# ska-sa/katsdpsigproc

Measured on AMD Instinct MI355X. Metric: visibility samples/s (baselines x channels) through full RFI flagger, higher is better.
Workload: dtype f32 amplitude / f64 deviations

## Files before the change

katsdpsigproc_amd/csrc/fused_common.h:

```cpp
#pragma once
#include <stdlib.h>

#include "bitplane.h"
#include "median_merge.h"
#include "median_window.h"

#ifndef FUSED_MAD_BITS
#define FUSED_MAD_BITS 1
#endif
#ifndef FUSED_STRIP
#define FUSED_STRIP 4
#endif
#define FUSED_THREADS (64 * FUSED_STRIP)
#define FUSED_MAD_NORMAL 1.4826

#ifdef KSP_DIAG_REALTIME
#define FUSED_DIAG_CLOCK() __builtin_amdgcn_s_memrealtime()
#else
#define FUSED_DIAG_CLOCK() __builtin_amdgcn_s_memtime()
#endif
#ifdef KSP_DIAG
#define FUSED_DIAG_STOP(p) ((p).debug_stop)
#define FUSED_DIAG_TRACE(p) ((p).trace)
#else
// ... 516 lines not shown
                                            int tiny = 0)
{
    static_assert(!HAVE_EXACT || R == 64, "exactness masks are 64 bits, one per sample of a lane");
    constexpr int NP = R / 2;
    const int c0 = lane * R;
    auto dv = [&](int j) -> float {
        float x = dev[j];
        asm("" : "+v"(x));
        return x;
    };
    unsigned kp[NP];
#pragma unroll
    for (int i = 0; i < NP; i++) {
        const unsigned a = __float_as_uint(dev[2 * i]) + 0xffffu;
        const unsigned b = __float_as_uint(dev[2 * i + 1]) + 0xffffu;
        kp[i] = __builtin_amdgcn_perm(b, a, 0x07060302u) & 0x7fff7fffu;
    }
    int zeros;
    if constexpr (R != 64) zeros = count_less16<NP>(kp, 1);
    auto stamp = [&](int i) {
        if (trace != nullptr && lane == 0) trace[i] = FUSED_DIAG_CLOCK();
    };
    stamp(8);
    if (debug_stop == 31) return (double)(kp[0] + kp[NP - 1]);
    const int total = 64 * R;
    unsigned K = 0;
    int below_bin = 0, in_bin;
    int rank2 = 0, rank = 0;
    int zeros_keys = 0;
    unsigned eq0 = 0, eq1 = 0;
    if constexpr (R == 64) {
        unsigned np[32];
#pragma unroll
        for (int i = 0; i < 32; i++) np[i] = kp[i] ^ 0x7fff7fffu;
        transpose_bits32(np);
        stamp(9);
        {
            unsigned z0 = np[0], z1 = np[16];
#pragma unroll
            for (int b = 1; b < 15; b++) {
                z0 &= np[b];
                z1 &= np[16 + b];
            }
            zeros = ksp_wave_sum_dpp(__popc(z0) + __popc(z1));
        }
        zeros_keys = zeros;
        if (ksp_any(tiny != 0)) zeros -= ksp_wave_sum_dpp(tiny);
        if (zeros == total) return __builtin_nan("");
        rank2 = total + zeros;
        rank = rank2 / 2;
        if (rank < zeros_keys) return 0x1p-150 * FUSED_MAD_NORMAL;
        eq0 = eq1 = 0xffffffffu;
        auto step2 = [&](int hi, int lo) {
            const unsigned a0 = eq0 & np[hi], a1 = eq1 & np[16 + hi];
            const unsigned z00_0 = a0 & np[lo], z00_1 = a1 & np[16 + lo];
            const unsigned z01_0 = a0 ^ z00_0, z01_1 = a1 ^ z00_1;
            const unsigned b0 = eq0 ^ a0, b1 = eq1 ^ a1;
            const unsigned z10_0 = b0 & np[lo], z10_1 = b1 & np[16 + lo];
            const unsigned z11_0 = b0 ^ z10_0, z11_1 = b1 ^ z10_1;
            int s01 = (__popc(z00_0) + __popc(z00_1)) | ((__popc(z01_0) + __popc(z01_1)) << 16);
            int c10 = __popc(z10_0) + __popc(z10_1);
            ksp_wave_sum2_dpp(s01, c10);
            const int n1 = below_bin + (s01 & 0xffff), n2 = n1 + (s01 >> 16), n3 = n2 + c10;
            const bool g1 = n1 <= rank, g2 = n2 <= rank, g3 = n3 <= rank;
            K |= (unsigned)((int)g1 + (int)g2 + (int)g3) << lo;
            below_bin = g3 ? n3 : g2 ? n2 : g1 ? n1 : below_bin;
            eq0 = g3 ? z11_0 : g2 ? z10_0 : g1 ? z01_0 : z00_0;
            eq1 = g3 ? z11_1 : g2 ? z10_1 : g1 ? z01_1 : z00_1;
        };
        auto step1 = [&](int bit) {
            const unsigned z0 = eq0 & np[bit], z1 = eq1 & np[16 + bit];
            const int c = below_bin + ksp_wave_sum_dpp(__popc(z0) + __popc(z1));
            const bool take = c <= rank;
            K |= take ? (1u << bit) : 0u;
            below_bin = take ? c : below_bin;
            eq0 = take ? (eq0 ^ z0) : z0;
            eq1 = take ? (eq1 ^ z1) : z1;
        };
#if FUSED_MAD_BITS == 1
        bool hinted = false;
        if (top_hint != nullptr && *top_hint >= 0) {
            const unsigned h = (unsigned)*top_hint;
            unsigned e0 = 0xffffffffu, e1 = 0xffffffffu;
            int lb = 0;
#pragma unroll
            for (int bit = 14; bit >= 7; bit--) {
                const unsigned z0 = e0 & np[bit], z1 = e1 & np[16 + bit];
                if ((h >> (bit - 7)) & 1) {
                    lb += __popc(z0) + __popc(z1);
                    e0 ^= z0;
                    e1 ^= z1;
                } else {
                    e0 = z0;
                    e1 = z1;
                }
            }
            int cnt = __popc(e0) + __popc(e1);
            ksp_wave_sum2_dpp(lb, cnt);
            if (lb <= rank && rank < lb + cnt) {
                hinted = true;
                K = h << 7;
                below_bin = lb;
                eq0 = e0;
                eq1 = e1;
            }
        }
        if (hinted) {
#pragma unroll
            for (int bit = 6; bit >= 0; bit--) step1(bit);
        } else {
#pragma unroll
            for (int bit = 14; bit >= 0; bit--) step1(bit);
        }
        if (top_hint != nullptr) *top_hint = (int)(K >> 7);
#else
#pragma unroll
        for (int bit = 14; bit >= 2; bit -= 2) step2(bit, bit - 1);
        step1(0);
#endif
        in_bin = ksp_wave_sum_dpp(__popc(eq0) + __popc(eq1));
    } else {
        zeros_keys = zeros;
        if (ksp_any(tiny != 0)) zeros -= ksp_wave_sum(tiny);
        if (zeros == total) return __builtin_nan("");
        rank2 = total + zeros;
        rank = rank2 / 2;
        if (rank < zeros_keys) return 0x1p-150 * FUSED_MAD_NORMAL;
        for (int bit = 14; bit >= 0; bit--) {
            const unsigned test = K | (1u << bit);
            const int c = count_less16<NP>(kp, test);
            if (c <= rank) {
                K = test;
                below_bin = c;
            }
        }
        in_bin = count_less16<NP>(kp, K + 1) - below_bin;
    }
    const bool even = !(rank2 & 1);
    stamp(10);
    if (debug_stop == 32) return (double)(K + below_bin);
    auto key_of = [&](int j) -> unsigned {
        return min((__float_as_uint(dv(j)) & 0x7fffffffu) + 0xffffu, 0x7fffffffu) >> 16;
    };
    auto bin_mask = [&](unsigned key) -> unsigned long long {
        unsigned long long m = 0;
#pragma unroll
        for (int j = 0; j < R; j++)
            if (key_of(j) == key) m |= 1ull << j;
        return m;
    };
    int r = rank - below_bin;
    unsigned long long cand = 0;
    const bool narrowed = in_bin > LIST_CAP;
    if (narrowed) {
        const unsigned first = ((K - 1) << 16) + 1u;
        unsigned offs = 0;
        int below = below_bin;
        for (int bit = 15; bit >= 0; bit--) {
            const unsigned test = first + (offs | (1u << bit));
            int c = 0;
#pragma unroll
            for (int j = 0; j < R; j++) c += (__float_as_uint(dv(j)) & 0x7fffffffu) < test;
            c = ksp_wave_sum(c);
            if (c <= rank) {
                offs |= 1u << bit;
                below = c;
            }
        }
        const unsigned cur = first + offs;
        cand = 0;
#pragma unroll
        for (int j = 0; j < R; j++)
            if ((__float_as_uint(dv(j)) & 0x7fffffffu) == cur) cand |= 1ull << j;
        in_bin = ksp_wave_sum(__popcll(cand));
        r = rank - below;
        below_bin = below;
        if (in_bin > LIST_CAP) {
            auto each = [&](auto &&f) {
                unsigned long long todo = cand;
                while (__any(todo != 0)) {
                    const bool has = todo != 0;
                    const int j = has ? __ffsll((long long)todo) - 1 : 0;
                    todo &= todo - 1;
                    const double x = fabs(exact_dev<WIDTH>(c0 + j, fetch));
                    if (has) f(x);
                }
            };
            double lo = __builtin_inf(), hi = 0.0;
            each([&](double x) {
                lo = fmin(lo, x);
                hi = fmax(hi, x);
            });
            lo = ksp_wave_min(lo);
            hi = ksp_wave_max(hi);
            double xk = lo, prev = lo;
            if (lo != hi) {
                const unsigned long long base = (unsigned long long)__double_as_longlong(lo);
                const unsigned long long span = (unsigned long long)__double_as_longlong(hi) - base;
                unsigned long long offs = 0;
                int below_k = 0;
                for (int bit = 63 - __clzll((long long)span); bit >= 0; bit--) {
                    const unsigned long long test = base + (offs | (1ull << bit));
                    int c = 0;
                    each([&](double x) {
                        c += (unsigned long long)__double_as_longlong(x) < test;
                    });
                    c = ksp_wave_sum(c);
                    if (c <= r) {
                        offs |= 1ull << bit;
                        below_k = c;
                    }
                }
                xk = __longlong_as_double((long long)(base + offs));
                prev = xk;
                if (even && r >= 1 && below_k == r) {
                    double m = 0.0;
                    each([&](double x) { m = (x < xk) ? fmax(m, x) : m; });
                    prev = ksp_wave_max(m);
                }
            }
            if (even && r == 0) {
                float b32 = 0.0f;
#pragma unroll
                for (int j = 0; j < R; j++) {
                    const float a = fabsf(dv(j));
                    b32 = (__float_as_uint(a) < cur) ? fmaxf(b32, a) : b32;
                }
                b32 = ksp_wave_max(b32);
                unsigned long long bm = 0;
#pragma unroll
                for (int j = 0; j < R; j++)
                    if (fabsf(dv(j)) == b32) bm |= 1ull << j;
                const int n2 = gather_exact<WIDTH>(bm, c0, list, 0, LIST_CAP, fetch);
                double below_max = 0.0;
                for (int i = lane; i < min(n2, LIST_CAP); i += 64) below_max = fmax(below_max, list[i]);
                below_max = ksp_wave_max(below_max);
                __builtin_amdgcn_wave_barrier();
                if (n2 > LIST_CAP) {
                    unsigned long long todo = bm;
                    double m = 0.0;
                    while (__any(todo != 0)) {
                        const bool has = todo != 0;
                        const int j = has ? __ffsll((long long)todo) - 1 : 0;
                        todo &= todo - 1;
                        const double x = fabs(exact_dev<WIDTH>(c0 + j, fetch));
                        m = has ? fmax(m, x) : m;
                    }
                    below_max = ksp_wave_max(m);
                }
                prev = below_max;
            }
            if (even) xk = (xk + prev) / 2.0;
            return xk * FUSED_MAD_NORMAL;
        }
    }
    double xk, prev;
    bool have_prev;
    if (!narrowed && in_bin <= 64) {
        int *lc = (int *)list;
        int n = 0;
        auto place = [&](bool hit, int channel) {
            const unsigned long long m = ksp_ballot(hit);
            const int pos = n + __builtin_amdgcn_mbcnt_hi((unsigned)(m >> 32),
                                                         __builtin_amdgcn_mbcnt_lo((unsigned)m, 0));
            if (hit) lc[pos] = channel;
            n += __popcll(m);
        };
        double x;
        bool ranked = false;
        unsigned *lv = (unsigned *)lc + 128;
        static_assert(LIST_CAP * 2 >= 128 + 64 + 8, "candidate values behind the channel numbers");
        if constexpr (R == 64 && HAVE_EXACT) {
            const int mine = __popc(eq0) + __popc(eq1);
            const int incl = ksp_wave_scan_dpp(mine);
            n = __builtin_amdgcn_readlane(incl, 63);
            int pos = incl - mine;
            unsigned h0 = eq0, h1 = eq1;
            while (ksp_any((h0 | h1) != 0)) {
                const bool has = (h0 | h1) != 0;
                int j = 0;
                if (h0) {
                    j = 2 * (__ffs((int)h0) - 1);
                    h0 &= h0 - 1;
                } else if (h1) {
                    j = 2 * (__ffs((int)h1) - 1) + 1;
                    h1 &= h1 - 1;
                }
                const float v = ksp_select_dev<R>(dev, j);
                if (has) {
                    lc[pos] = (c0 + j) | (((exact >> j) & 1) ? (int)0x80000000 : 0);
                    lv[pos] = __float_as_uint(v) & 0x7fffffffu;
                    pos++;
                }
            }
            if (lane < 8) lv[n + lane] = 0xffffffffu;
            __builtin_amdgcn_fence(__ATOMIC_RELEASE, "wavefront");
            __builtin_amdgcn_wave_barrier();
            const int slot = lane < n ? lane : 0;
            const int e0 = lc[slot];
            const unsigned a32 = lv[slot];
            x = (double)__uint_as_float(a32);
            const bool inexact = lane < n && e0 >= 0;
            stamp(11);
            if (debug_stop == 33) return x;
            if (ksp_any(inexact)) {
                const double xe = fabs(exact_dev<WIDTH>(e0 & 0x7fffffff, fetch));
                x = inexact ? xe : x;
            } else {
                unsigned k32, p32;
                rank_list_u32(lv, a32, n, r, lane, k32, p32, have_prev);
                xk = (double)__uint_as_float(k32);
                prev = (double)__uint_as_float(p32);
                ranked = true;
            }
        } else {
            if constexpr (R == 64) {
                const int mine = __popc(eq0) + __popc(eq1);
                const int incl = ksp_wave_scan_dpp(mine);
                n = __builtin_amdgcn_readlane(incl, 63);
                int pos = incl - mine;
                unsigned h0 = eq0, h1 = eq1;
                while (h0 | h1) {
                    if (h0) {
                        lc[pos++] = c0 + 2 * (__ffs((int)h0) - 1);
                        h0 &= h0 - 1;
                    } else {
                        lc[pos++] = c0 + 2 * (__ffs((int)h1) - 1) + 1;
                        h1 &= h1 - 1;
                    }
                }
            } else {
#pragma unroll
                for (int j = 0; j < R; j++) place(key_of(j) == K, c0 + j);
            }
            __builtin_amdgcn_fence(__ATOMIC_RELEASE, "wavefront");
            __builtin_amdgcn_wave_barrier();
            const int c = lc[lane < n ? lane : 0];
            stamp(11);
            if (debug_stop == 33) return (double)c;
            x = fabs(exact_dev<WIDTH>(c, fetch));
        }
        stamp(12);
        if (!ranked) rank_lanes64(x, n, r, lane, xk, prev, have_prev);
        stamp(13);
        __builtin_amdgcn_wave_barrier();
    } else {
        gather_exact<WIDTH>(narrowed ? cand : bin_mask(K), c0, list, 0, LIST_CAP, fetch);
        rank_in_list(list, in_bin, r, lane, xk, prev, have_prev);
        __builtin_amdgcn_wave_barrier();
    }
    if (even && !have_prev) {
        int k2 = -1;
#pragma unroll
        for (int j = 0; j < R; j++) {
            const int kj = (int)key_of(j);
            k2 = (kj < (int)K) ? max(k2, kj) : k2;
        }
        k2 = wave_max_int(k2);
        const bool below_is_tiny = k2 <= 0;
        unsigned long long bm = bin_mask((unsigned)(below_is_tiny ? 0 : k2));
        float b32 = 0.0f;
#pragma unroll
        for (int j = 0; j < R; j++)
            if ((bm >> j) & 1) b32 = fmaxf(b32, fabsf(dv(j)));
        b32 = ksp_wave_max(b32);
        unsigned long long top = 0;
#pragma unroll
        for (int j = 0; j < R; j++)
            if (((bm >> j) & 1) && fabsf(dv(j)) == b32) top |= 1ull << j;
        bool recompute = true;
        if (below_is_tiny) {
            prev = 0x1p-150;
            recompute = false;
        }
        if constexpr (HAVE_EXACT) {
            if (recompute && !ksp_any((top & ~exact) != 0)) {
                prev = (double)b32;
                recompute = false;
            }
        }
        if (recompute) {
            const int n2 = gather_exact<WIDTH>(top, c0, list, 0, LIST_CAP, fetch);
            double below_max = 0.0;
            for (int i = lane; i < min(n2, LIST_CAP); i += 64) below_max = fmax(below_max, list[i]);
            prev = ksp_wave_max(below_max);
            __builtin_amdgcn_wave_barrier();
            if (n2 > LIST_CAP) {
                double m = 0.0;
                while (__any(top != 0)) {
                    const bool has = top != 0;
                    const int j = has ? __ffsll((long long)top) - 1 : 0;
                    top &= top - 1;
                    const double x = fabs(exact_dev<WIDTH>(c0 + j, fetch));
                    m = has ? fmax(m, x) : m;
                }
                prev = ksp_wave_max(m);
            }
        }
    }
    stamp(14);
    if (even) xk = (xk + prev) / 2.0;
    return xk * FUSED_MAD_NORMAL;
}

template <int WIDTH, class Fetch>
__device__ __noinline__ double exact_dev_call(int c, Fetch fetch)
{
    return exact_dev<WIDTH>(c, fetch);
}

template <int WIDTH, class Fetch>
__device__ __forceinline__ unsigned long long threshold_wide(const FusedParams &p,
                                                             const float (&dev)[64],
                                                             unsigned long long fl,
                                                             unsigned long long ge, double t1,
                                                             bool positive, int lane, int C,
                                                             Fetch &&fetch)
{
    const int c0 = lane * 64;
    float nmax = 0.0f;
#pragma unroll
    for (int j = 0; j < 64; j++) nmax = fmaxf(nmax, -dev[j]);
    nmax = ksp_wave_max(nmax);
    float U[64];
    unsigned Nb[16];
#pragma unroll
    for (int j = 0; j < 64; j++) U[j] = dev[j];
#pragma unroll
    for (int q = 0; q < 16; q++) Nb[q] = 0;
    int lvl = -1;
    float umax = 0.0f;
    bool counted = false;
    auto level = [&](auto s_) {
        constexpr int s = decltype(s_)::value;
        ksp_static_for<s>([&](auto r_) {
            constexpr int r = decltype(r_)::value;
            const float e = __shfl_down(U[r], 1, 64);
#pragma unroll
            for (int j = r; j + s < 64; j += s) U[j] += U[j + s];
            U[r + 64 - s] += e;
        });
        if (counted) {
            if constexpr (s >= 4) {
                constexpr int sq = s / 4;
                ksp_static_for<sq>([&](auto r_) {
                    constexpr int r = decltype(r_)::value;
                    const unsigned e = (unsigned)__shfl_down((int)Nb[r], 1, 64);
#pragma unroll
                    for (int q = r; q + sq < 16; q += sq) Nb[q] += Nb[q + sq];
                    Nb[r + 16 - sq] += e;
                });
            } else {
                const unsigned e = (unsigned)__shfl_down((int)Nb[0], 1, 64);
#pragma unroll
                for (int q = 0; q < 16; q++)
                    Nb[q] += __builtin_amdgcn_alignbyte(q + 1 < 16 ? Nb[(q + 1) % 16] : e, Nb[q], s);
            }
        }
    };
#pragma unroll 1
    for (int k = 0; k < p.n_windows; k++) {
        if (positive && !ksp_any((ge & ~fl) != 0)) break;
        const int w = 1 << k;
        const double scale = k == 0 ? p.scales[0] : k == 1 ? p.scales[1] : k == 2 ? p.scales[2]
                           : k == 3 ? p.scales[3] : k == 4 ? p.scales[4] : k == 5 ? p.scales[5]
                           : k == 6 ? p.scales[6] : p.scales[7];
        const float thrf = (float)(t1 * scale);
        const float limf = __fmul_rn(thrf, (float)w);
        const double limit = (double)limf;
        if (positive && lvl >= 0 && umax < thrf) continue;
        if (lvl < 0) {
            counted = ksp_any(fl != 0);
            {
                const unsigned f_lo = (unsigned)fl, f_hi = (unsigned)(fl >> 32);
#pragma unroll
                for (int j = 0; j < 64; j++)
                    U[j] = (((j < 32 ? f_lo : f_hi) >> (j & 31)) & 1u) ? 0.0f : dev[j];
            }
            float m = U[0];
#pragma unroll
            for (int j = 1; j < 64; j++) m = fmaxf(m, U[j]);
            umax = ksp_wave_max(m);
            if (counted) {
#pragma unroll
                for (int q = 0; q < 16; q++)
                    Nb[q] = ((((unsigned)(fl >> (4 * q))) & 0xfu) * 0x00204081u) & 0x01010101u;
            }
            lvl = 0;
            if (positive && umax < thrf) continue;
        }
        while (lvl < k) {
            switch (lvl) {
            case 0: level(std::integral_constant<int, 1>{}); break;
            case 1: level(std::integral_constant<int, 2>{}); break;
            case 2: level(std::integral_constant<int, 4>{}); break;
            case 3: level(std::integral_constant<int, 8>{}); break;
            case 4: level(std::integral_constant<int, 16>{}); break;
            case 5: level(std::integral_constant<int, 32>{}); break;
            default: level(std::integral_constant<int, 64>{}); break;
            }
            lvl++;
        }
        const int nvalid = C - w + 1 - c0;
        const unsigned long long valid = nvalid >= 64 ? ~0ull : nvalid <= 0 ? 0ull : ((1ull << nvalid) - 1);
        unsigned long long hits = 0, unsure = valid;
        if (positive) {
            unsigned h_lo = 0, h_hi = 0, m_lo = 0, m_hi = 0;
            const float c = (float)w * nmax * 0x1p-18f + (float)w * 0x1p-149f;
            if (counted) {
                const unsigned wq = (unsigned)w * 0x01010101u;
                auto one = [&](auto j_, unsigned &h, unsigned &m) {
                    constexpr int j = decltype(j_)::value;
                    const unsigned left = wq - Nb[j / 4];
                    const float rem = (float)((left >> (8 * (j % 4))) & 0xffu);
                    const float T = rem * thrf;
                    const float hi = __builtin_fmaf(T, 1.0f + 0x1p-18f, c);
                    float lo = __builtin_fmaf(T, 1.0f - 0x1p-18f, -c);
                    lo = (rem == 0.0f) ? __builtin_inff() : lo;
                    h = 2 * h + (U[j] > hi);
                    m = 2 * m + (U[j] > lo);
                };
                ksp_static_for<32>([&](auto i_) { one(std::integral_constant<int, 31 - decltype(i_)::value>{}, h_lo, m_lo); });
                ksp_static_for<32>([&](auto i_) { one(std::integral_constant<int, 63 - decltype(i_)::value>{}, h_hi, m_hi); });
            } else {
                const float hi = __builtin_fmaf(limf, 1.0f + 0x1p-18f, c);
                const float lo = __builtin_fmaf(limf, 1.0f - 0x1p-18f, -c);
#pragma unroll
                for (int j = 31; j >= 0; j--) {
                    h_lo = 2 * h_lo + (U[j] > hi);
                    m_lo = 2 * m_lo + (U[j] > lo);
                }
#pragma unroll
                for (int j = 63; j >= 32; j--) {
                    h_hi = 2 * h_hi + (U[j] > hi);
                    m_hi = 2 * m_hi + (U[j] > lo);
                }
            }
            hits = (((unsigned long long)h_hi << 32) | h_lo) & valid;
            unsure = (((unsigned long long)m_hi << 32) | m_lo) & valid & ~hits;
        }
        if (ksp_any(unsure != 0)) {
            const unsigned long long f1 = __shfl_down(fl, 1, 64), f2 = __shfl_down(fl, 2, 64);
            while (ksp_any(unsure != 0)) {
                const bool has = unsure != 0;
                const int j = has ? __ffsll((long long)unsure) - 1 : 0;
                unsure &= unsure - 1;
                double s = 0.0;
                for (int m = 0; m < w; m++) {
                    const int jj = j + m;
                    const unsigned long long fw = jj < 64 ? fl : jj < 128 ? f1 : f2;
                    const bool sub = (fw >> (jj & 63)) & 1;
                    const double x = exact_dev_call<WIDTH>(c0 + jj, fetch);
                    s += sub ? (double)thrf : x;
                }
                if (has && s > limit) hits |= 1ull << j;
            }
            lvl = -1;
        }
        if (!ksp_any(hits != 0)) continue;
        auto suffix_or = [](unsigned long long t) {
            t |= t >> 1; t |= t >> 2; t |= t >> 4; t |= t >> 8; t |= t >> 16; t |= t >> 32;
            return t;
        };
        unsigned long long add = hits;
        for (int s = 1; s < w && s < 64; s <<= 1) add |= add << s;
        unsigned long long h1 = __shfl_up(hits, 1, 64), h2 = __shfl_up(hits, 2, 64);
        if (lane < 1) h1 = 0;
        if (lane < 2) h2 = 0;
        if (w > 64) {
            add |= h1 ? ~0ull : 0ull;
            add |= suffix_or(h2 >> 1);
        } else if (w > 1) {
            add |= suffix_or(h1 >> (65 - w));
        }
        if (ksp_any((add & ~fl) != 0)) {
            fl |= add;
            lvl = -1;
        }
    }
    return fl;
}


template <int R, int WIDTH, int MAXK = 4, class Fetch>
__device__ __forceinline__ unsigned long long threshold_flags(const FusedParams &p,
                                                              const float (&dev)[R], float dmax,
                                                              double noise64, int lane, int C,
                                                              Fetch &&fetch)
{
    static_assert(R <= 64, "flag mask is 64 bits");
    const int c0 = lane * R;
    unsigned long long fl = 0;
    if (p.threshold_kind == KSP_THRESHOLD_SIMPLE) {
        const double thr = p.n_sigma * noise64;
        if (__any((double)dmax * (1.0 + 0x1p-23) > thr)) {
            unsigned long long unsure = 0;
#pragma unroll
            for (int j = 0; j < R; j++) {
                const double d = (double)dev[j];
                const double slack = fabs(d) * 0x1p-23 + 0x1p-149;
                if (d - slack > thr)
                    fl |= 1ull << j;
                else if (d + slack > thr)
                    unsure |= 1ull << j;
            }
            while (__any(unsure != 0)) {
// ... 165 lines not shown
```

katsdpsigproc_amd/csrc/ring_kernel.h:

```cpp
#pragma once
#include "fused_common.h"

#ifndef RING_STOP
#define RING_STOP 0
#endif
#define RING_THREADS 512
#define RING_STRIP 8
#define RING_NSLOT 32
#ifndef RING_G
#define RING_G 4
#endif
#ifndef RING_PRIO
#define RING_PRIO 0
#endif
#ifndef RING_STAGGER
#define RING_STAGGER 0
#endif
#define RING_SLOT_BYTES 4096
#define RING_LIST_DOUBLES 256
#define RING_XCD_GROUP 8

struct RingLayout {
    static constexpr size_t RING_BYTES = (size_t)RING_NSLOT * RING_SLOT_BYTES;
    static constexpr size_t LIST_BYTES = sizeof(double) * RING_LIST_DOUBLES * RING_STRIP;
    static constexpr size_t CTRL_BYTES = 64;
    static constexpr size_t LDS_BYTES = RING_BYTES + LIST_BYTES + CTRL_BYTES;
};

#ifdef RING_TRACE
#define RING_TRACE_STRIPS 24
#define RING_TRACE_SLOTS 16
__device__ unsigned long long ring_trace_buf[256 * 8 * RING_TRACE_STRIPS * RING_TRACE_SLOTS];
#endif

#define RING_WORK_LIST 2
#define RING_WORK_DONE 10

__device__ __forceinline__ int ring_strip_of(int x, int t)
{
    return ((t / RING_XCD_GROUP) * 8 + x) * RING_XCD_GROUP + (t % RING_XCD_GROUP);
}

__device__ __forceinline__ int ring_take(unsigned *work, int x, int n_strips, int t0)
{
    for (int k = 0; k < 8; k++) {
        const int xx = (x + k) & 7;
        const int t = t0 + (int)atomicAdd(&work[RING_WORK_LIST + xx], 1u);
        const int s = ring_strip_of(xx, t);
        if (s < n_strips) return s;
    }
    return -1;
}

__device__ __forceinline__ float ring_from_next(float v, float edge, int lane)
{
    const float r = __shfl_down(v, 1, 64);
    return lane == 63 ? edge : r;
}
__device__ __forceinline__ float ring_from_prev(float v, float edge, int lane)
{
    const float r = __shfl_up(v, 1, 64);
    return lane == 0 ? edge : r;
}

template <int WIDTH>
__global__ __launch_bounds__(RING_THREADS) void flagger_ring_kernel(const FusedParams p)
{
    constexpr int R = 64, W = WIDTH, H = WIDTH / 2;
    constexpr int G = RING_G, NSLOT = RING_NSLOT, STEPS = 64, NCHUNK = STEPS / G;
    constexpr int K = NSLOT / G;
    constexpr int PER_CHUNK = G / 2;
    static_assert(W % 2 == 1 && W <= 13 && 2 * H <= G * 3, "merging median only");
    typedef __attribute__((address_space(3))) void lds_void;
    extern __shared__ __attribute__((aligned(16))) char lds[];
    const int tid = threadIdx.x, lane = tid & 63;
    const int wave = __builtin_amdgcn_readfirstlane(tid >> 6);
    const int C = p.channels;
    double *list = (double *)(lds + RingLayout::RING_BYTES) + wave * RING_LIST_DOUBLES;
    int *ctrl = (int *)(lds + RingLayout::RING_BYTES + RingLayout::LIST_BYTES);
    const unsigned lds_base = (unsigned)(size_t)(lds_void *)lds;

    const int q = wave & 3, par = wave >> 2;
    const int rl = lane >> 2;
    const int chunk16 = (lane & 3) ^ ((rl >> 2) & 3);
    const size_t row_bytes = (size_t)p.vis_stride * 8;
    const unsigned lane_off = (unsigned)((size_t)(16 * q + rl) * 64 * row_bytes + (size_t)chunk16 * 16);
    const int pp = wave >> 1, hh = wave & 1;
    const int l16 = lane & 15;
    const unsigned rd_off = (lane >> 4) * 1024 + l16 * 64 + ((pp ^ ((l16 >> 2) & 3)) * 16) + 8 * hh;
    typedef const __attribute__((address_space(3))) char lds_cchar;
    typedef const __attribute__((address_space(3))) unsigned long long lds_cu64;
    lds_cchar *lds3 = (lds_cchar *)(lds_void *)lds;

    unsigned long long run_src = 0;
    const unsigned long long rb2 = 2 * (unsigned long long)row_bytes;
    const unsigned piece_base = __builtin_amdgcn_readfirstlane(lds_base + q * 1024);
    auto issue = [&](int slot) {
        unsigned pb = piece_base;
        asm volatile("" : "+s"(pb));
        const unsigned dst = pb + (unsigned)(slot + par) * RING_SLOT_BYTES;
        unsigned keep;
        asm volatile("s_mov_b32 %0, m0\n\ts_mov_b32 m0, %3\n\ts_nop 0\n\t"
                     "global_load_lds_dwordx4 %1, %2\n\ts_mov_b32 m0, %0"
                     : "=&s"(keep) : "v"(lane_off), "s"(run_src), "s"(dst) : "memory");
        run_src += rb2;
    };
    auto strip_base = [&](int strip) -> const char * {
        return (const char *)p.vis + (size_t)strip * (RING_STRIP * 8);
    };

    const int xcd = blockIdx.x & 7;
    const int per_list = (int)gridDim.x >> 3;
    const int t0 = p.n_static * per_list;
    auto static_strip = [&](int k) { return ring_strip_of(xcd, k * per_list + ((int)blockIdx.x >> 3)); };
    if (tid == 0) {
        int s0 = 0 < p.n_static ? static_strip(0) : ring_take(p.work, xcd, p.n_strips, t0);
        int s1 = -1;
        if (s0 >= 0) s1 = 1 < p.n_static ? static_strip(1) : ring_take(p.work, xcd, p.n_strips, t0);
        ctrl[0] = s0;
        ctrl[1] = s1;
    }
    __syncthreads();
    int cur = __builtin_amdgcn_readfirstlane(ctrl[0]), nxt = __builtin_amdgcn_readfirstlane(ctrl[1]);
    int k_strip = 0;
    auto finish = [&]() {
        if (tid == 0 && atomicAdd(&p.work[RING_WORK_DONE], 1u) == gridDim.x - 1u) {
#pragma unroll
            for (int k = RING_WORK_LIST; k <= RING_WORK_DONE; k++) p.work[k] = 0;
        }
    };
    if (cur < 0) {
        finish();
        return;
    }
#if RING_STAGGER > 0
    if ((blockIdx.x >> 3) & 1) {
#pragma unroll
        for (int i = 0; i < RING_STAGGER; i++) __builtin_amdgcn_s_sleep(127);
    }
#endif
    auto start_of = [&](int strip) -> unsigned long long {
        const unsigned long long a = (unsigned long long)strip_base(strip) + (unsigned long long)par * row_bytes;
        return ((unsigned long long)(unsigned)__builtin_amdgcn_readfirstlane((unsigned)(a >> 32)) << 32) |
               (unsigned long long)(unsigned)__builtin_amdgcn_readfirstlane((unsigned)a);
    };
    run_src = start_of(cur);
#pragma unroll
    for (int j = 0; j < NSLOT; j += 2) issue(j);
    float2 zz[2][G];
    auto read_chunk = [&](int chunk, float2 (&z)[G]) {
        unsigned ro = rd_off + ((chunk * G) % NSLOT) * RING_SLOT_BYTES;
        asm volatile("" : "+v"(ro));
#pragma unroll
        for (int g = 0; g < G; g++) {
            const unsigned long long w = *(lds_cu64 *)(lds3 + ro + g * RING_SLOT_BYTES);
            z[g] = make_float2(__uint_as_float((unsigned)w), __uint_as_float((unsigned)(w >> 32)));
        }
    };
    auto convert_chunk = [&](const float2 (&z)[G], float *a, unsigned &um) {
        static_assert(G == 4, "the pin below names four results");
        unsigned key = ~0u;
#pragma unroll
        for (int g = 0; g < G; g++) key &= ksp_abs_range_key(z[g].x, z[g].y);
#pragma unroll
        for (int g = 0; g < G; g += 2)
            ksp_abs_c64_inrange_x2(z[g].x, z[g].y, z[g + 1].x, z[g + 1].y, a[g], a[g + 1]);
        asm volatile("" : "+v"(a[0]), "+v"(a[1]), "+v"(a[2]), "+v"(a[3]));
        if (ksp_any((key & KSP_ABS_RANGE_BIT) == 0)) {
#pragma unroll
            for (int g = 0; g < G; g++) {
                a[g] = ksp_abs_c64(z[g].x, z[g].y);
                um = max(um, __float_as_uint(a[g]));
            }
        }
    };
    float amp_nxt[G];
    unsigned umax_nxt = 0;
    {
        constexpr int AH0 = (K - 1) * PER_CHUNK;
        __builtin_amdgcn_s_waitcnt(0x0070 | (AH0 & 15) | ((AH0 >> 4) << 14));
        __syncthreads();
        read_chunk(0, zz[0]);
        convert_chunk(zz[0], amp_nxt, umax_nxt);
    }
    const float nanv = __builtin_nanf("");
    const float2 *visf = (const float2 *)p.vis;

#if RING_PRIO == 1
    if (wave >= 4) __builtin_amdgcn_s_setprio(1);
#endif
    int mad_hint = -1;
    const int lane_id = lane;
#ifdef RING_TRACE
    int trace_it = 0;
#define RING_STAMP(i)                                                                              \
    do {                                                                                           \
        if (lane_id == 0 && trace_it < RING_TRACE_STRIPS && blockIdx.x < 256)                      \
            ring_trace_buf[((blockIdx.x * 8 + wave) * RING_TRACE_STRIPS + trace_it) * RING_TRACE_SLOTS + (i)] =   \
                __builtin_amdgcn_s_memtime();                                                      \
    } while (0)
#else
#define RING_STAMP(i) do { } while (0)
#endif
    for (;;) {
        int lane = lane_id;
        asm volatile("" : "+v"(lane));
        const int bl = cur * RING_STRIP + wave;
        const bool more = nxt >= 0;
        const unsigned long long start_nxt = start_of(more ? nxt : cur);
        auto fetch = [&](int c) -> float {
            const bool inside = c >= 0 && c < C;
            const int cc = inside ? c : 0;
            const float2 v = visf[(size_t)cc * p.vis_stride + bl];
            float a = ksp_abs_c64(v.x, v.y);
            return inside ? a : nanv;
        };
        RING_STAMP(0);
#ifdef RING_TRACE
        unsigned long long wait_dma = 0, wait_bar = 0;
        if (lane_id == 0 && trace_it < RING_TRACE_STRIPS && blockIdx.x < 256)
            ring_trace_buf[((blockIdx.x * 8 + wave) * RING_TRACE_STRIPS + trace_it) * RING_TRACE_SLOTS + 4] = __builtin_amdgcn_s_memrealtime();
#endif
        float amp[STEPS];
        unsigned umax = umax_nxt;
        umax_nxt = 0;
#pragma unroll
        for (int g = 0; g < G; g++) amp[g] = amp_nxt[g];
        auto load_chunk = [&](auto more_, auto c_) {
            constexpr bool MORE = decltype(more_)::value;
            constexpr int c = decltype(c_)::value;
            constexpr int AH = (K - 3) * PER_CHUNK;
#ifdef RING_TRACE
            unsigned long long w0;
            asm volatile("s_memtime %0\n\ts_waitcnt lgkmcnt(0)" : "=s"(w0));
#endif
            if constexpr (MORE || (c + K - 1) * G + G <= STEPS)
                __builtin_amdgcn_s_waitcnt(0x0070 | (AH & 15) | ((AH >> 4) << 14));
            else
                __builtin_amdgcn_s_waitcnt(0x0070);
#ifdef RING_TRACE
            unsigned long long w1;
            asm volatile("s_memtime %0\n\ts_waitcnt lgkmcnt(0)" : "=s"(w1));
#endif
#ifndef RING_NOSYNC
            __syncthreads();
#endif
#ifdef RING_TRACE
            unsigned long long w2;
            asm volatile("s_memtime %0\n\ts_waitcnt lgkmcnt(0)" : "=s"(w2));
            wait_dma += w1 - w0;
            wait_bar += w2 - w1;
#endif
            ksp_static_for<G / 2>([&](auto u_) {
                constexpr int j = c * G + 2 * decltype(u_)::value + NSLOT;
                if constexpr (j < STEPS) {
                    issue(j % NSLOT);
                } else if constexpr (MORE) {
                    if constexpr (j == STEPS) run_src = start_nxt;
                    issue(j % NSLOT);
                }
            });
            if constexpr (c == 0) read_chunk(1, zz[1]);
            if constexpr (c + 2 < NCHUNK || (MORE && c + 2 == NCHUNK)) read_chunk(c + 2, zz[c & 1]);
#if RING_PRIO == 2
            if ((c + (wave >> 2)) & 1)
                __builtin_amdgcn_s_setprio(1);
            else
                __builtin_amdgcn_s_setprio(0);
#endif
            if constexpr (c + 1 < NCHUNK)
                convert_chunk(zz[(c + 1) & 1], &amp[(c + 1) * G], umax);
            else if constexpr (MORE)
                convert_chunk(zz[(c + 1) & 1], amp_nxt, umax_nxt);
        };

        float dev[R];
        float dmax;
        unsigned ex_a = 0, ex_b = 0;
        int tiny = 0;
        auto note_exact = [&](unsigned &acc, float x, float m, float d) {
            unsigned t;
            asm("v_min_u32 %1, %2, %3\n\tv_or_b32 %1, 0x7fffff, %1\n\t"
                "v_cmp_ge_f32 vcc, %1, |%4|\n\tv_addc_co_u32 %0, vcc, %0, %0, vcc"
                : "+v"(acc), "=&v"(t)
                : "v"(__float_as_uint(x)), "v"(__float_as_uint(m)), "v"(d)
                : "vcc");
        };
        auto stream = [&](auto more_) __attribute__((always_inline)) {
#if RING_STOP == 1
            dmax = 0.f;
            ksp_static_for<NCHUNK>([&](auto c_) {
                load_chunk(more_, c_);
                constexpr int c = decltype(c_)::value;
#pragma unroll
                for (int g = 0; g < G; g++) {
                    dev[c * G + g] = amp[c * G + g];
                    dmax += amp[c * G + g];
                }
            });
#else
            MergeMedian<R, W> mm;
            mm.pinf = __builtin_inff();
            mm.ninf = -__builtin_inff();
            asm volatile("" : "+v"(mm.pinf), "+v"(mm.ninf));
            const float pinf = mm.pinf, ninf = mm.ninf;
            const bool first = lane == 0, last = lane == 63;
            dmax = ninf;
            float rh[H];
            auto X = [&](auto i_) -> float {
                constexpr int i = decltype(i_)::value;
                if constexpr (i < STEPS) {
                    if constexpr (i % G == 0) load_chunk(more_, std::integral_constant<int, i / G>{});
                    return amp[i];
                } else {
                    if constexpr (i == STEPS) {
#pragma unroll
                        for (int k = 0; k < H; k++)
                            rh[k] = ring_from_next(amp[k], (k & 1) ? ninf : pinf, lane);
                    }
                    return rh[i - STEPS];
                }
            };
            constexpr int RV = R - H;
            constexpr int STAGES = (RV + W - 1) / W;
            using MM = MergeMedian<R, W>;
            float cur_b[W];
            ksp_static_for<W>([&](auto k_) { cur_b[decltype(k_)::value] = X(k_); });
            ksp_static_for<STAGES>([&](auto m_) {
                constexpr int m = decltype(m_)::value;
                float S[MM::S_SIZE];
                S[MM::off(W - 1)] = cur_b[W - 1];
                ksp_static_for<W - 1>([&](auto u_) {
                    constexpr int t = W - 2 - decltype(u_)::value;
                    mm.template insert<W - 1 - t>(&S[MM::off(t + 1)], cur_b[t], &S[MM::off(t)]);
                });
                float P[W], nxt_b[W];
                ksp_static_for<W>([&](auto t_) {
                    constexpr int t = decltype(t_)::value;
                    constexpr int jv = m * W + t;
                    if constexpr (jv < RV) {
                        constexpr int j = jv + H;
                        if constexpr (t >= 1) {
                            nxt_b[t - 1] = X(std::integral_constant<int, (m + 1) * W + t - 1>{});
                            if constexpr (t == 1)
                                P[0] = nxt_b[0];
                            else
                                mm.template insert<t - 1>(P, nxt_b[t - 1], P);
                        }
                        const float med = mm.template rank<W - t, t, H>(&S[MM::off(t)], P);
                        const float xc = (t + H < W) ? cur_b[t + H < W ? t + H : 0] : nxt_b[t + H >= W ? t + H - W : 0];
                        float d = xc - med;
                        constexpr bool right_odd = j + H >= R && ((j + H - R + 1) & 1);
                        if constexpr (right_odd) {
                            const float lo = mm.template rank<W - t, t, H - 1>(&S[MM::off(t)], P);
                            if (last) {
                                const double dd = (double)xc - ((double)lo + (double)med) * 0.5;
                                d = (float)dd;
                                tiny += (d == 0.0f && dd != 0.0);
                            }
                        }
                        asm volatile("" : "+v"(d));
                        if constexpr (jv < 32)
                            note_exact(ex_a, xc, med, d);
                        else
                            note_exact(ex_b, xc, med, d);
                        if constexpr (jv & 1)
                            asm("v_max3_f32 %0, %0, %1, %2" : "+v"(dmax) : "v"(dev[j - 1]), "v"(d));
                        else if constexpr (jv == RV - 1)
                            dmax = mm.vmax(dmax, d);
                        dev[j] = d;
                    }
                });
                if constexpr (m + 1 < STAGES) {
                    ksp_static_for<W>([&](auto k_) {
                        constexpr int k = decltype(k_)::value;
                        constexpr int i = (m + 1) * W + k;
                        constexpr bool have = (m * W + k + 1 < RV) && (k + 1 < W);
                        if constexpr (!have) {
                            if constexpr (i < R + H)
                                nxt_b[k] = X(std::integral_constant<int, i>{});
                            else
                                nxt_b[k] = pinf;
                        }
                    });
#pragma unroll
                    for (int k = 0; k < W; k++) cur_b[k] = nxt_b[k];
                }
            });
            if constexpr (H >= 1) {
                float L[H];
#pragma unroll
                for (int k = 0; k < H; k++)
                    L[k] = ring_from_prev(amp[STEPS - H + k], ((H - k) & 1) ? pinf : ninf, lane);
                constexpr auto soff = [](int j) { return j * H - j * (j - 1) / 2; };
                float SL[H * (H + 1) / 2];
                SL[soff(H - 1)] = L[H - 1];
                ksp_static_for<H - 1>([&](auto u_) {
                    constexpr int j = H - 2 - decltype(u_)::value;
                    mm.template insert<H - 1 - j>(&SL[soff(j + 1)], L[j], &SL[soff(j)]);
                });
                float PL[2 * H];
                PL[0] = amp[0];
                ksp_static_for<H>([&](auto k_) {
                    constexpr int k = decltype(k_)::value + 1;
                    mm.template insert<k>(PL, amp[k], PL);
                });
                ksp_static_for<H>([&](auto j_) {
                    constexpr int j = decltype(j_)::value;
                    if constexpr (j >= 1) mm.template insert<j + H>(PL, amp[j + H], PL);
                    const float med = mm.template rank<H - j, j + H + 1, H>(&SL[soff(j)], PL);
                    const float xc = amp[j];
                    float d = xc - med;
                    if constexpr ((H - j) & 1) {
                        const float lo = mm.template rank<H - j, j + H + 1, H - 1>(&SL[soff(j)], PL);
                        if (first) {
                            const double dd = (double)xc - ((double)lo + (double)med) * 0.5;
                            d = (float)dd;
                            tiny += (d == 0.0f && dd != 0.0);
                        }
                    }
                    note_exact(ex_b, xc, med, d);
                    dmax = mm.vmax(dmax, d);
                    dev[j] = d;
                });
            }
#endif
        };
        if (more)
            stream(std::true_type{});
        else
            stream(std::false_type{});
        RING_STAMP(1);
#ifdef RING_TRACE
        if (lane_id == 0 && trace_it < RING_TRACE_STRIPS && blockIdx.x < 256) {
            ring_trace_buf[((blockIdx.x * 8 + wave) * RING_TRACE_STRIPS + trace_it) * RING_TRACE_SLOTS + 5] = wait_dma;
            ring_trace_buf[((blockIdx.x * 8 + wave) * RING_TRACE_STRIPS + trace_it) * RING_TRACE_SLOTS + 6] = wait_bar;
        }
#endif
        unsigned long long exact;
        {
            const unsigned ra = __builtin_bitreverse32(ex_a), rb = __builtin_bitreverse32(ex_b);
            exact = ((unsigned long long)ra << H) |
                    ((unsigned long long)(rb & ((1u << (32 - H)) - 1u)) << (H + 32)) |
                    (unsigned long long)(rb >> (32 - H));
            unsigned long long first_odd = 0, last_odd = 0;
#pragma unroll
            for (int j = 0; j < H; j++)
                if ((H - j) & 1) first_odd |= 1ull << j;
#pragma unroll
            for (int j = R - H; j < R; j++)
                if ((j + H - R + 1) & 1) last_odd |= 1ull << j;
            if (lane == 0) exact &= ~first_odd;
            if (lane == 63) exact &= ~last_odd;
        }
        if (ksp_any(umax >= 0x7f800000u)) {
            float a2[R + 2 * H];
            int c_first = lane * R - H;
            asm volatile("" : "+v"(c_first));
#pragma unroll
            for (int i = 0; i < R + 2 * H; i++) a2[i] = fetch(c_first + i);
            tiny = 0;
            median_phase_src<R, W>([&](int i) { return a2[i + H]; }, dev, dmax, &tiny);
            exact = 0;
        }
        const bool ticket = more && k_strip + 2 >= p.n_static;
        unsigned t_own = 0;
        if (tid == 0 && ticket) t_own = atomicAdd(&p.work[RING_WORK_LIST + xcd], 1u);

#if RING_STOP == 1 || RING_STOP == 2
        {
            float acc = dmax;
#pragma unroll
            for (int j = 0; j < R; j++) acc += dev[j];
            if (acc == 12345.678f && p.noise != nullptr) p.noise[bl] = acc;
        }
#else
        const double noise64 = mad_noise<R, W, RING_LIST_DOUBLES, true>(dev, lane, list, fetch, RING_STOP > 30 ? RING_STOP : 0,
#ifdef RING_TRACE
                                                                      (trace_it < RING_TRACE_STRIPS && blockIdx.x < 256)
                                                                          ? &ring_trace_buf[((blockIdx.x * 8 + wave) * RING_TRACE_STRIPS + trace_it) * RING_TRACE_SLOTS]
                                                                          : nullptr,
#else
                                                                      nullptr,
#endif
                                                                      exact, &mad_hint, tiny);
        if (lane == 0 && p.noise != nullptr) p.noise[bl] = (float)noise64;
        RING_STAMP(2);
#if RING_STOP == 3 || RING_STOP > 30
        if (noise64 == 12345.678 && p.noise != nullptr) p.noise[bl] = dmax;
#else
        const unsigned long long fl = threshold_flags<R, W>(p, dev, dmax, noise64, lane, C, fetch);
        write_flags(p, fl, lane * R, bl, C);
        RING_STAMP(3);
#endif
#endif

#ifdef RING_TRACE
        if (lane_id == 0 && trace_it < RING_TRACE_STRIPS && blockIdx.x < 256)
            ring_trace_buf[((blockIdx.x * 8 + wave) * RING_TRACE_STRIPS + trace_it) * RING_TRACE_SLOTS + 7] = (unsigned long long)cur + 1;
        trace_it++;
#endif
        if (!more) break;
        cur = nxt;
        if (!ticket) {
            nxt = static_strip(k_strip + 2);
#ifdef RING_END_SYNC
            __syncthreads();
#endif
        } else {
            if (tid == 0) {
                int take = ring_strip_of(xcd, t0 + (int)t_own);
                if (take >= p.n_strips) take = ring_take(p.work, (xcd + 1) & 7, p.n_strips, t0);
                ctrl[2] = take;
            }
            __syncthreads();
            nxt = __builtin_amdgcn_readfirstlane(ctrl[2]);
            __syncthreads();
        }
        k_strip++;
    }
    finish();
}

inline bool ring_supported(const FusedParams &p, int width)
{
    return p.channels == 4096 && width % 2 == 1 && width >= 3 && width <= 13 && !p.is_amplitude &&
           p.flags_mode == KSP_FLAGS_NONE && p.deviations == nullptr && p.work != nullptr &&
           p.baselines >= RING_STRIP && (p.vis_stride % 2) == 0 &&
           (p.threshold_kind != KSP_THRESHOLD_SUM || p.n_windows <= 4) &&
           (size_t)p.vis_stride * 8 * 4096 < 0x7fffff00ull;
}

template <int WIDTH>
inline int launch_ring(int device, hipStream_t s, const FusedParams &p_in, int n_cu, hipEvent_t ev0,
                       hipEvent_t ev1)
{
    FusedParams p = p_in;
    p.n_strips = p.baselines / RING_STRIP;
    auto kern = flagger_ring_kernel<WIDTH>;
    static std::atomic<bool> attr_set[64];
    if (device < 0 || device >= 64 || !attr_set[device].load(std::memory_order_acquire)) {
        KSP_CHECK(hipFuncSetAttribute((const void *)kern, hipFuncAttributeMaxDynamicSharedMemorySize,
                                      (int)RingLayout::LDS_BYTES));
        if (device >= 0 && device < 64) attr_set[device].store(true, std::memory_order_release);
    }
    const int grid = p.n_strips < n_cu ? p.n_strips : n_cu;
    p.n_static = 0;
    if (grid % 8 == 0 && p.n_strips / grid >= 3) {
        const int by_share = p.n_strips / grid - 2;
        const int by_range = (8 * (p.n_strips / 64)) / (grid / 8);
        p.n_static = by_share < by_range ? by_share : by_range;
    }
#ifndef RING_STATIC
    p.n_static = 0;
#endif
#ifdef RING_TRACE
    {
        void *tb = nullptr;
        KSP_CHECK(hipGetSymbolAddress(&tb, HIP_SYMBOL(ring_trace_buf)));
        KSP_CHECK(hipMemsetAsync(tb, 0, sizeof(ring_trace_buf), s));
    }
#endif
    if (ev0 != nullptr)
        hipExtLaunchKernelGGL(kern, dim3(grid), dim3(RING_THREADS), RingLayout::LDS_BYTES, s, ev0, ev1,
                              0, p);
    else
        hipLaunchKernelGGL(kern, dim3(grid), dim3(RING_THREADS), RingLayout::LDS_BYTES, s, p);
    KSP_LAUNCH_CHECK();
#ifdef RING_TRACE
    if (const char *path = getenv("KSP_RING_TRACE")) {
        KSP_CHECK(hipStreamSynchronize(s));
        const size_t n = sizeof(ring_trace_buf);
        void *host = malloc(n);
        KSP_CHECK(hipMemcpyFromSymbol(host, HIP_SYMBOL(ring_trace_buf), n));
        FILE *f = fopen(path, "wb");
        if (f != nullptr) {
            fwrite(host, 1, n, f);
            fclose(f);
        }
        free(host);
    }
#endif
    return 0;
}
```

Before: 366.9 billion.

## Use paired ds_read2st64 LDS reads with explicit waitcnt in the ring kernel

Replaces the four separate 64-bit LDS reads per chunk with two ds_read2st64_b64 instructions using immediate offsets, and adds explicit lgkmcnt waits so reads for a later chunk overlap with conversion of the current one. The per-wave slot offset is folded into the base address register to shorten the DMA issue path. It also drops one instruction from the exact-deviation check, which changes its threshold, and adds a trace write of the inexact count. The hand-managed waitcnt ordering is fragile if compiler scheduling changes, and the altered comparison may change flagging results.

```diff
diff --git a/katsdpsigproc_amd/csrc/fused_common.h b/katsdpsigproc_amd/csrc/fused_common.h
--- a/katsdpsigproc_amd/csrc/fused_common.h
+++ b/katsdpsigproc_amd/csrc/fused_common.h
@@ -842,6 +842,7 @@
             x = (double)__uint_as_float(a32);
             const bool inexact = lane < n && e0 >= 0;
             stamp(11);
+            if (trace != nullptr && lane == 0) trace[15] = 1ull + (unsigned long long)__popcll(ksp_ballot(inexact));
             if (debug_stop == 33) return x;
             if (ksp_any(inexact)) {
                 const double xe = fabs(exact_dev<WIDTH>(e0 & 0x7fffffff, fetch));
diff --git a/katsdpsigproc_amd/csrc/ring_kernel.h b/katsdpsigproc_amd/csrc/ring_kernel.h
--- a/katsdpsigproc_amd/csrc/ring_kernel.h
+++ b/katsdpsigproc_amd/csrc/ring_kernel.h
@@ -88,17 +88,15 @@
     const int pp = wave >> 1, hh = wave & 1;
     const int l16 = lane & 15;
     const unsigned rd_off = (lane >> 4) * 1024 + l16 * 64 + ((pp ^ ((l16 >> 2) & 3)) * 16) + 8 * hh;
-    typedef const __attribute__((address_space(3))) char lds_cchar;
-    typedef const __attribute__((address_space(3))) unsigned long long lds_cu64;
-    lds_cchar *lds3 = (lds_cchar *)(lds_void *)lds;
 
     unsigned long long run_src = 0;
     const unsigned long long rb2 = 2 * (unsigned long long)row_bytes;
-    const unsigned piece_base = __builtin_amdgcn_readfirstlane(lds_base + q * 1024);
+    const unsigned piece_base = __builtin_amdgcn_readfirstlane(lds_base + q * 1024 + par * RING_SLOT_BYTES);
+    unsigned piece_strip = piece_base;
     auto issue = [&](int slot) {
-        unsigned pb = piece_base;
+        unsigned pb = piece_strip;
         asm volatile("" : "+s"(pb));
-        const unsigned dst = pb + (unsigned)(slot + par) * RING_SLOT_BYTES;
+        const unsigned dst = pb + (unsigned)slot * RING_SLOT_BYTES;
         unsigned keep;
         asm volatile("s_mov_b32 %0, m0\n\ts_mov_b32 m0, %3\n\ts_nop 0\n\t"
                      "global_load_lds_dwordx4 %1, %2\n\ts_mov_b32 m0, %0"
@@ -148,15 +146,31 @@
 #pragma unroll
     for (int j = 0; j < NSLOT; j += 2) issue(j);
     float2 zz[2][G];
-    auto read_chunk = [&](int chunk, float2 (&z)[G]) {
-        unsigned ro = rd_off + ((chunk * G) % NSLOT) * RING_SLOT_BYTES;
-        asm volatile("" : "+v"(ro));
-#pragma unroll
-        for (int g = 0; g < G; g++) {
-            const unsigned long long w = *(lds_cu64 *)(lds3 + ro + g * RING_SLOT_BYTES);
-            z[g] = make_float2(__uint_as_float((unsigned)w), __uint_as_float((unsigned)(w >> 32)));
-        }
+    const unsigned rd_addr = lds_base + rd_off;
+    typedef unsigned ring_u32x4 __attribute__((ext_vector_type(4)));
+    ring_u32x4 zq[2][2];
+    auto read_chunk = [&](auto chunk_, auto set_) {
+        static_assert(G == 4 && RING_SLOT_BYTES == 8 * 512, "two reads of two steps, 8 offset units per slot");
+        constexpr int o = ((decltype(chunk_)::value * G) % NSLOT) * 8, set = decltype(set_)::value;
+        static_assert(o + 24 <= 255, "8-bit offsets");
+        const unsigned base = rd_addr;
+        ring_u32x4 &r0 = zq[set][0], &r1 = zq[set][1];
+        asm volatile("ds_read2st64_b64 %0, %2 offset0:%3 offset1:%4\n\t"
+                     "ds_read2st64_b64 %1, %2 offset0:%5 offset1:%6"
+                     : "=&v"(r0), "=&v"(r1)
+                     : "v"(base), "n"(o), "n"(o + 8), "n"(o + 16), "n"(o + 24)
+                     : "memory");
     };
+    auto reads_done = [&](auto set_, auto younger_) {
+        constexpr int set = decltype(set_)::value;
+        ring_u32x4 &r0 = zq[set][0], &r1 = zq[set][1];
+        asm volatile("s_waitcnt lgkmcnt(%2)" : "+v"(r0), "+v"(r1) : "n"(decltype(younger_)::value));
+        zz[set][0] = make_float2(__uint_as_float(r0.x), __uint_as_float(r0.y));
+        zz[set][1] = make_float2(__uint_as_float(r0.z), __uint_as_float(r0.w));
+        zz[set][2] = make_float2(__uint_as_float(r1.x), __uint_as_float(r1.y));
+        zz[set][3] = make_float2(__uint_as_float(r1.z), __uint_as_float(r1.w));
+    };
+#define RING_INT(i) std::integral_constant<int, (i)>{}
     auto convert_chunk = [&](const float2 (&z)[G], float *a, unsigned &um) {
         static_assert(G == 4, "the pin below names four results");
         unsigned key = ~0u;
@@ -180,7 +194,8 @@
         constexpr int AH0 = (K - 1) * PER_CHUNK;
         __builtin_amdgcn_s_waitcnt(0x0070 | (AH0 & 15) | ((AH0 >> 4) << 14));
         __syncthreads();
-        read_chunk(0, zz[0]);
+        read_chunk(RING_INT(0), RING_INT(0));
+        reads_done(RING_INT(0), RING_INT(0));
         convert_chunk(zz[0], amp_nxt, umax_nxt);
     }
     const float nanv = __builtin_nanf("");
@@ -205,6 +220,8 @@
     for (;;) {
         int lane = lane_id;
         asm volatile("" : "+v"(lane));
+        piece_strip = piece_base;
+        asm volatile("" : "+s"(piece_strip));
         const int bl = cur * RING_STRIP + wave;
         const bool more = nxt >= 0;
         const unsigned long long start_nxt = start_of(more ? nxt : cur);
@@ -260,8 +277,9 @@
                     issue(j % NSLOT);
                 }
             });
-            if constexpr (c == 0) read_chunk(1, zz[1]);
-            if constexpr (c + 2 < NCHUNK || (MORE && c + 2 == NCHUNK)) read_chunk(c + 2, zz[c & 1]);
+            if constexpr (c == 0) read_chunk(RING_INT(1), RING_INT(1));
+            if constexpr (c + 2 < NCHUNK || (MORE && c + 2 == NCHUNK)) read_chunk(RING_INT(c + 2), RING_INT(c & 1));
+            if constexpr (c == 0) reads_done(RING_INT(1), RING_INT(2));
 #if RING_PRIO == 2
             if ((c + (wave >> 2)) & 1)
                 __builtin_amdgcn_s_setprio(1);
@@ -272,6 +290,7 @@
                 convert_chunk(zz[(c + 1) & 1], &amp[(c + 1) * G], umax);
             else if constexpr (MORE)
                 convert_chunk(zz[(c + 1) & 1], amp_nxt, umax_nxt);
+            if constexpr (c + 2 < NCHUNK || (MORE && c + 2 == NCHUNK)) reads_done(RING_INT(c & 1), RING_INT(0));
         };
 
         float dev[R];
@@ -280,7 +299,7 @@
         int tiny = 0;
         auto note_exact = [&](unsigned &acc, float x, float m, float d) {
             unsigned t;
-            asm("v_min_u32 %1, %2, %3\n\tv_or_b32 %1, 0x7fffff, %1\n\t"
+            asm("v_min_u32 %1, %2, %3\n\t"
                 "v_cmp_ge_f32 vcc, %1, |%4|\n\tv_addc_co_u32 %0, vcc, %0, %0, vcc"
                 : "+v"(acc), "=&v"(t)
                 : "v"(__float_as_uint(x)), "v"(__float_as_uint(m)), "v"(d)
```

Result: slower. 343.1 billion (-6.5%).
